# joncampbell123/composite-video-simulator

Measured on AMD Instinct MI355X. Metric: frames/sec (output frames = fields; 720x486 NTSC, preset '-vhs'; steady-state pipelined throughput, 4 steps in flight), higher is better.
Workload: dtype f64; 1 GPU; 720x486 30fps 10s colour-bars clip, preset '-vhs': 300 frames -> 600 fields per GPU per step, frame-round-robin over 1 GPU(s); steps_in_flight=4, mode=exact (bit-identical to the reference: fp64, no FMA contraction)

## Files before the change

### composite-video-simulator_amd/csrc/lane_rand.hpp

```cpp
#pragma once
#include <stdint.h>

#ifndef DEV
#define DEV __device__ __forceinline__
#endif

struct LaneRand {
    uint32_t p3, p2, p1;
    int slot;
    DEV void init(uint32_t *ring, const uint32_t *state, int stride, int lane)
    {
        for (int j = 0; j < 31; j++) ring[j * 64 + lane] = state[(size_t)j * stride];
        p3 = ring[28 * 64 + lane];
        p2 = ring[29 * 64 + lane];
        p1 = ring[30 * 64 + lane];
        slot = 0;
    }
    DEV uint32_t next(uint32_t *ring, int lane)
    {
#ifdef NTSC_AB_NORAND
        (void)ring; (void)lane;
        p3 = p3 * 1664525u + 1013904223u;
        return p3 >> 1;
#endif
        const uint32_t v = ring[slot * 64 + lane] + p3;
        ring[slot * 64 + lane] = v;
        p3 = p2; p2 = p1; p1 = v;
        slot = (slot == 30) ? 0 : slot + 1;
        return v >> 1;
    }
};

DEV void jump61(const uint32_t *__restrict__ c, const uint32_t *__restrict__ w, uint32_t (&o)[31])
{
    uint32_t cc[31], ww[61];
#pragma unroll
    for (int k = 0; k < 31; k++) cc[k] = c[k];
#pragma unroll
    for (int i = 0; i < 61; i++) ww[i] = w[i];
#pragma unroll
    for (int j = 0; j < 31; j++) {
        uint32_t acc = 0;
#pragma unroll
        for (int k = 0; k < 31; k++) acc += cc[k] * ww[j + k];
        o[j] = acc;
    }
}
```

### composite-video-simulator_amd/csrc/ntsc_device.hpp

```cpp
#pragma once
#include <cstdint>
#include "glibc_rand.hpp"

namespace ntscsim {

struct DevParams {
    int W, H;
    int Lslot;
    int nfields;
    int R;
    int Rpad;
    int ntsc;
    int phase_mode, phase_off;
    int in_lp;
    int out_lp;
    int amp, amp_back;
    Magic31 m_amp, m_amp_back;
    int noise_k;  Magic31 m_noise;
    int cnoise_k; Magic31 m_cnoise;
    int pnoise_k; Magic31 m_pnoise;
    int loss;
    int hs, hs_noise_on;
    double hs_point, hs_phase, hs_pn;
    int nocolor;
    int vhs, vblend, svideo, cdelay;
    int pre_on;
    double pre_gain, a_pre;
    double a_in_i, a_in_q, a_tv, a_vl, a_vc, a_sh;
    double sharpen;
    int src_al16, dst_al16;
    int warm_luma, warm_chroma;
    int variant;
    int ghost_taps, ghost_delay[4], ghost_gain[4];
};

struct FieldDev {
    const uint8_t *src;
    uint8_t *dst;
    int32_t src_ls, dst_ls;
    uint32_t field, flags;
    uint64_t fieldno;
    uint32_t rng[61];
    uint32_t _pad;
};
static_assert(sizeof(FieldDev) == 288, "FieldDev layout");

struct GeomDev {
    const uint32_t *lskip;
    const uint32_t *pskip;
    const uint32_t *jrow;
    const int32_t  *jwarm;
    const uint32_t *sstart;
    const double   *ptab;
};

}
```

### composite-video-simulator_amd/csrc/ntsc_kernels.hip

```cpp
#include <hip/hip_runtime.h>
#include <stdint.h>
#include "ntsc_device.hpp"

#pragma clang fp contract(off)

namespace ntscsim {

#define DEV __device__ __forceinline__

DEV int sdiv2(int n) { return (n + (int)((unsigned)n >> 31)) >> 1; }
DEV int sdiv4(int n) { return (n + ((n >> 31) & 3)) >> 2; }
DEV unsigned udiv31(unsigned n, const Magic31 &m) { return __umulhi(n, m.mul) >> m.shift; }
DEV unsigned umod31(unsigned n, const Magic31 &m) { return n - udiv31(n, m) * m.div; }
DEV int noise_next(int n, unsigned draw, const Magic31 &m, int k)
{
#ifdef NTSC_NOISE_UPDATE_OLD
    return sdiv2(n + (int)umod31(draw, m) - k);
#else
    int nk = -k;
    asm("" : "+s"(nk));
    unsigned t = ((unsigned)n + draw) + (unsigned)nk;
    asm("" : "+v"(t));
    return sdiv2((int)(t - udiv31(draw, m) * m.div));
#endif
}
DEV int sdivm(int n, const Magic31 &m)
{
    if (m.mul == 0) return n;
    const unsigned a = (unsigned)(n < 0 ? -n : n);
    const int q = (int)udiv31(a, m);
    return n < 0 ? -q : q;
}

DEV unsigned scan_phase(const DevParams &P, unsigned y, uint64_t fieldno)
{
// ... 123 lines not shown
            y += 2;
            shy++;
        }
    }

    if (P.pnoise_k || P.loss) {
        jump61(G.pskip + field * 31, fd.rng, st);
        g.init(ring, st, lane);
        if (P.pnoise_k) {
            int n = 0;
            for (int k = 0; k < L; k++) {
                n += (int)umod31(g.next(ring, lane), P.m_pnoise) - P.pnoise_k;
                n = sdiv2(n);
                pn_noise[(size_t)f * P.Lslot + k] = n;
            }
        }
        if (P.loss) {
            for (int k = 0; k < L; k++)
                dropout[(size_t)f * P.Lslot + k] = (g.next(ring, lane) % 100000U) < (unsigned)P.loss;
        }
    }
}

__global__ __launch_bounds__(64) void k_field_setup(DevParams P, GeomDev G,
                                                    const FieldDev *__restrict__ fields,
                                                    int *__restrict__ hs_shift,
                                                    int *__restrict__ pn_noise,
                                                    int *__restrict__ dropout)
{
    __shared__ uint32_t ring[31 * 64];
    field_setup_body(P, G, fields, hs_shift, pn_noise, dropout, ring, (int)blockIdx.x);
}

DEV void row_states_body(const DevParams &P, const GeomDev &G, const FieldDev *__restrict__ fields,
                         uint32_t *__restrict__ rs_luma, int *__restrict__ n0_luma,
                         uint32_t *__restrict__ rs_chroma, int *__restrict__ n0_u, int *__restrict__ n0_v,
                         uint32_t *ring, int block, int stream)
{
    const int lane = threadIdx.x;
    const int rho = block * 64 + lane;
    if (rho >= P.R) return;
    if (stream == 0 ? !P.noise_k : !P.cnoise_k) return;
    const int f = rho / P.Lslot, k = rho - f * P.Lslot;
    const FieldDev &fd = fields[f];
    const unsigned par = fd.field & 1u;
    if (k >= field_rows(P, par)) return;

    const size_t jidx = ((size_t)(stream * 2 + par) * P.Lslot + k);
    const int warm = G.jwarm[jidx];
    const int K = stream == 0 ? P.noise_k : P.cnoise_k;
    const Magic31 M = stream == 0 ? P.m_noise : P.m_cnoise;
    const long long cpr = P.variant ? 2ll * (P.W / 2) : 2ll * P.W;
    const long long start = stream == 0 ? (long long)k * P.W : cpr * k;
    const bool exact = (long long)warm == start;

    uint32_t st[31];
    SetupRand g;
    jump61(G.jrow + jidx * 31, fd.rng, st);
    g.init(ring, st, lane);

    int lo0 = exact ? 0 : -K, hi0 = exact ? 0 : K;
    int lo1 = stream == 0 ? 0 : lo0, hi1 = stream == 0 ? 0 : hi0;
    if (stream == 0) {
        for (int i = 0; i < warm; i++) {
            const int d = (int)umod31(g.next(ring, lane), M) - K;
            lo0 = sdiv2(lo0 + d); hi0 = sdiv2(hi0 + d);
        }
    } else {
        for (int i = 0; i < warm; i += 2) {
            int d = (int)umod31(g.next(ring, lane), M) - K;
            lo0 = sdiv2(lo0 + d); hi0 = sdiv2(hi0 + d);
            d = (int)umod31(g.next(ring, lane), M) - K;
            lo1 = sdiv2(lo1 + d); hi1 = sdiv2(hi1 + d);
        }
    }
    if (lo0 != hi0 || lo1 != hi1) {
        jump61(G.sstart + (size_t)(stream * 2 + par) * 31, fd.rng, st);
        g.init(ring, st, lane);
        lo0 = lo1 = 0;
        if (stream == 0) {
            for (long long i = 0; i < start; i++)
                lo0 = sdiv2(lo0 + (int)umod31(g.next(ring, lane), M) - K);
        } else {
            for (long long i = 0; i < start; i += 2) {
                lo0 = sdiv2(lo0 + (int)umod31(g.next(ring, lane), M) - K);
                lo1 = sdiv2(lo1 + (int)umod31(g.next(ring, lane), M) - K);
            }
        }
    }

    uint32_t *rs = stream == 0 ? rs_luma : rs_chroma;
    int q = g.slot;
    for (int j = 0; j < 31; j++) {
        rs[(size_t)j * P.Rpad + rho] = ring[q * 64 + lane];
        q = (q == 30) ? 0 : q + 1;
    }
    if (stream == 0) n0_luma[rho] = lo0;
    else { n0_u[rho] = lo0; n0_v[rho] = lo1; }
}

__global__ __launch_bounds__(64) void k_row_states(DevParams P, GeomDev G,
                                                   const FieldDev *__restrict__ fields,
                                                   uint32_t *__restrict__ rs_luma,
                                                   int *__restrict__ n0_luma,
                                                   uint32_t *__restrict__ rs_chroma,
                                                   int *__restrict__ n0_u, int *__restrict__ n0_v)
{
    __shared__ uint32_t ring[31 * 64];
    row_states_body(P, G, fields, rs_luma, n0_luma, rs_chroma, n0_u, n0_v, ring, (int)blockIdx.x, (int)blockIdx.y);
}

DEV void field_part_body(const DevParams &P, const GeomDev &G, const FieldDev *__restrict__ fields,
                         int *__restrict__ hs_shift, int *__restrict__ pn_noise, int *__restrict__ dropout,
                         uint32_t *ring, int f, int part)
{
    const int lane = threadIdx.x;
    const FieldDev &fd = fields[f];
    const unsigned field = fd.field & 1u;
    const int L = field_rows(P, field);
    const bool on = part == 0 ? P.hs != 0 : (part == 1 ? P.pnoise_k != 0 : P.loss != 0);
    if (!on) return;
    int *hs_row = hs_shift + (size_t)f * P.Lslot;
    if (part == 0)
        for (int k = lane; k < P.Lslot; k += 64) hs_row[k] = 0;
    if (part == 0) __builtin_amdgcn_s_waitcnt(0x0F70);
    if (part != 0 || P.hs_noise_on) {
        const uint32_t *c = (part == 0 ? G.lskip : G.pskip + (part == 2 ? 62 : 0)) + field * 31;
        if (lane < 31) {
            uint32_t acc = 0;
#pragma unroll
            for (int k = 0; k < 31; k++) acc += c[k] * fd.rng[lane + k];
// ... 789 lines not shown
```

### composite-video-simulator_amd/csrc/ntsc_key.hip

```cpp
#include <hip/hip_runtime.h>

#include <algorithm>
#include <cstdint>
#include <cstring>
#include <map>
#include <new>
#include <string>
#include <vector>

#include "key_host.hpp"
#include "ntscsim.h"
#include "ntsc_layer_frames.hpp"
#include "ntsc_px4.hpp"

namespace ntscsim {

#define KDEV __device__ __forceinline__

constexpr int KEY_FAST = NTSCSIM_KEY_FAST_LAYERS;
constexpr int KEY_THREADS = 256;
constexpr int KEY_DRAW_THREADS = 64;

struct KeyCfgLayer {
    uint32_t color;
    int32_t thr;
    uint32_t fade, xdivr, invert, noisekey;
};
struct KeyCfg { KeyCfgLayer l[KEY_FAST]; };

struct KeyLayerDev {
    const uint8_t *src;
    const uint32_t *bits;
    int32_t ls, _pad;
};

struct KeyRec {
    uint8_t *dst;
    const uint8_t *src[KEY_FAST];
    const uint32_t *bits[KEY_FAST];
    const KeyLayerDev *layers;
    int32_t src_ls[KEY_FAST];
    int32_t dst_ls;
    uint32_t vec;
    uint32_t _pad[2];
};

struct KeyJob {
    uint32_t st[31];
    uint32_t noisekey;
    uint32_t *bits;
};

struct KeyClip {
    uint8_t *const *ring;
    int32_t ring_ls, ri, delay, T;
};

#include "lane_rand.hpp"

__global__ __launch_bounds__(KEY_DRAW_THREADS) void k_key_draw(const KeyJob *__restrict__ jobs, const uint32_t *__restrict__ polys,
                                                               uint32_t lanes)
{
    __shared__ uint32_t ring[31 * 64];
    const int lane = threadIdx.x;
    const uint32_t j = blockIdx.x * KEY_DRAW_THREADS + lane;
    const uint32_t jj = j < lanes ? j : lanes - 1;
    const KeyJob &job = jobs[blockIdx.y];
    uint32_t w[61], c[31], st[31];
#pragma unroll
    for (int i = 0; i < 31; i++) w[i] = job.st[i];
#pragma unroll
    for (int i = 31; i < 61; i++) w[i] = w[i - 31] + w[i - 3];
#pragma unroll
    for (int k = 0; k < 31; k++) c[k] = polys[(size_t)k * lanes + jj];
    jump61(c, w, st);
#pragma unroll
    for (int i = 0; i < 31; i++) ring[i * 64 + lane] = st[i];
    LaneRand g;
    g.p3 = st[28]; g.p2 = st[29]; g.p1 = st[30];
    g.slot = 0;
    const uint32_t nk = job.noisekey;
    uint32_t *out = job.bits + (size_t)jj * KEY_RUN_WORDS;
#pragma unroll 1
    for (int wi = 0; wi < KEY_RUN_WORDS; wi++) {
        uint32_t word = 0;
#pragma unroll 4
        for (int b = 0; b < 32; b++) {
            const uint32_t r1 = g.next(ring, lane), r2 = g.next(ring, lane), r3 = g.next(ring, lane);
            const uint32_t x = (r1 * r2 * r3) % 20001u;
            word |= (x < nk ? 1u : 0u) << b;
// ... 596 lines not shown
```

### composite-video-simulator_amd/csrc/ntscsim_hip.hip

```cpp
#include <hip/hip_runtime.h>

#include <algorithm>
#include <cmath>
#include <cstdio>
#include <cstdlib>
#include <cstring>
#include <mutex>
#include <new>
#include <string>
#include <vector>

#include "ntscsim.h"
#include "ntsc_device.hpp"
#include "engine_host.hpp"

#include "ntsc_kernels.hip"
#include "ntsc_decode_fast.hip"
#include "ntsc_encode_fast.hip"
#include "ntsc_pipe.hip"
#include "ntsc422_kernels.hip"
#include "ntsc422_fused.hip"
#include "ntsc_scale.hip"
#include "ntsc_float.hpp"
#include "ntsc_stage.hpp"
// ... 20 lines not shown
        const hipError_t e = hipHostMalloc((void **)&bounce, CAP, hipHostMallocPortable);
        if (e != hipSuccess) { bounce = nullptr; return e; }
    }
    const unsigned char *s = static_cast<const unsigned char *>(src_host);
    unsigned char *d = static_cast<unsigned char *>(dst_dev);
    for (size_t off = 0; off < bytes; off += CAP) {
        const size_t n = bytes - off < CAP ? bytes - off : CAP;
        std::memcpy(bounce, s + off, n);
        const hipError_t e = hipMemcpy(d + off, bounce, n, hipMemcpyHostToDevice);
        if (e != hipSuccess) return e;
    }
    return hipSuccess;
}

template <typename T>
struct DevBuf {
    T *p = nullptr;
    size_t cap = 0;
    hipError_t ensure(size_t n)
    {
        if (n <= cap) return hipSuccess;
        if (p) { (void)hipFree(p); p = nullptr; cap = 0; }
        size_t want = n + n / 8 + 64;
        hipError_t e = hipMalloc((void **)&p, want * sizeof(T));
        if (e == hipSuccess) cap = want;
        return e;
    }
    void release() { if (p) (void)hipFree(p); p = nullptr; cap = 0; }
};

struct Geometry {
    int W = 0, H = 0, variant = 0;
    bool valid = false;
    DevBuf<uint32_t> lskip, pskip, jrow, sstart;
    DevBuf<int32_t> jwarm;
    uint64_t calls[2] = {0, 0};
};

}

struct SubmitEngine;
struct Host422Engine;
struct PinCache;

struct ntscsim_ctx {
    ntscsim_params prm;
    int device = 0;
    hipStream_t stream = nullptr;
    std::string err;
    uint64_t rng_pos = 0;

    bool have_state = false;
    uint64_t state_pos = 0;
    RandState state;
    struct Delta { uint64_t n; RandPoly p; };
    std::vector<Delta> deltas;

    std::vector<Geometry *> geoms;
    Geometry *geom_cur = nullptr;
    DevBuf<double> ptab;
    bool ptab_ready = false;

    DevBuf<FieldDev> fields;
    DevBuf<int> hs_shift, pn_noise, dropout, n0_luma, n0_u, n0_v, comp, comp_ghost, comp_vcr, tails;
    DevBuf<Field422Dev> fields422;
    DevBuf<uint8_t> recs422;
    DevBuf<uint32_t> scratch422;
    DevBuf<uint8_t> halo422;
// ... 143 lines not shown
    D.amp_back = p.subcarrier_amplitude_back;
    D.m_amp = magic31((uint32_t)D.amp);
    D.m_amp_back = magic31((uint32_t)D.amp_back);
    D.noise_k = p.video_noise;
    D.m_noise = magic31((uint32_t)(2 * p.video_noise + 1));
    D.cnoise_k = p.video_chroma_noise;
    D.m_cnoise = magic31((uint32_t)(2 * p.video_chroma_noise + 1));
    D.pnoise_k = p.video_chroma_phase_noise;
    D.m_pnoise = magic31((uint32_t)(2 * p.video_chroma_phase_noise + 1));
    D.loss = p.video_chroma_loss;
    D.hs = p.vhs_head_switching != 0;
    D.hs_noise_on = p.vhs_head_switching_phase_noise != 0;
    D.hs_point = p.vhs_head_switching_point;
    D.hs_phase = p.vhs_head_switching_phase;
    D.hs_pn = p.vhs_head_switching_phase_noise;
    D.nocolor = p.nocolor_subcarrier != 0;
    D.vhs = p.emulating_vhs != 0;
    D.vblend = p.vhs_chroma_vert_blend != 0;
    D.svideo = p.vhs_svideo_out != 0;
    double luma_cut = 2400000, chroma_cut = 320000;
    D.cdelay = 9;
    if (p.output_vhs_tape_speed == NTSCSIM_VHS_LP) { luma_cut = 1900000; chroma_cut = 300000; D.cdelay = 12; }
    if (p.output_vhs_tape_speed == NTSCSIM_VHS_EP) { luma_cut = 1400000; chroma_cut = 280000; D.cdelay = 14; }
    D.pre_on = (p.composite_preemphasis != 0 && p.composite_preemphasis_cut > 0);
    D.pre_gain = p.composite_preemphasis;
    D.a_pre = D.pre_on ? alpha_for(p.composite_preemphasis_cut) : 0;
    D.a_in_i = alpha_for(1300000);
    D.a_in_q = alpha_for(600000);
    D.a_tv = alpha_for(2600000);
    D.a_vl = alpha_for(luma_cut);
    D.a_vc = alpha_for(chroma_cut);
    D.a_sh = alpha_for(luma_cut * 4);
    D.sharpen = p.vhs_out_sharpen;
    D.warm_luma = 64;
    D.warm_chroma = 128;
    D.ghost_taps = p.ghost_taps;
    for (int k = 0; k < 4; k++) { D.ghost_delay[k] = p.ghost_delay[k]; D.ghost_gain[k] = p.ghost_gain[k]; }
}

static uint64_t chroma_stream_offset(const ntscsim_params &p, int W, int L)
{
    uint64_t o = 0;
    if (p.video_noise != 0) o += (uint64_t)W * L;
    if (p.vhs_head_switching && p.vhs_head_switching_phase_noise != 0) o += 4;
    return o;
}

static int build_geometry(ntscsim_ctx *c, int W, int H, const DevParams &D)
{
    for (Geometry *e : c->geoms)
        if (e->valid && e->W == W && e->H == H && e->variant == D.variant) { c->geom_cur = e; return NTSCSIM_OK; }
    if (c->geoms.size() >= 16) {
        HIPCHK(c, hipDeviceSynchronize());
        for (Geometry *e : c->geoms) {
            e->lskip.release(); e->pskip.release(); e->jrow.release(); e->sstart.release(); e->jwarm.release();
            delete e;
        }
        c->geoms.clear();
    }
    Geometry *gp = new (std::nothrow) Geometry();
    if (!gp) return NTSCSIM_E_NOMEM;
    c->geoms.push_back(gp);
    c->geom_cur = gp;
    Geometry &g = *gp;
    g.valid = false;
    const uint64_t cdraws = D.variant ? 2ull * (uint64_t)(W / 2) : 2ull * (uint64_t)W;
    const int Lslot = (H + 1) / 2;
    const int Lp[2] = {(H + 1) / 2, H / 2};
    std::vector<uint32_t> lskip(2 * 31), pskip(4 * 31), sstart(4 * 31), jrow((size_t)4 * Lslot * 31);
    std::vector<int32_t> jwarm((size_t)4 * Lslot);
    const RandPoly xW = rand_poly_pow((uint64_t)W), x2W = rand_poly_pow(cdraws);
    for (int par = 0; par < 2; par++) {
        const uint64_t off_hs = c->prm.video_noise != 0 ? (uint64_t)W * Lp[par] : 0;
        const uint64_t off_pn = chroma_stream_offset(c->prm, W, Lp[par]) +
                                (c->prm.video_chroma_noise != 0 ? cdraws * Lp[par] : 0);
        const RandPoly a = rand_poly_pow(off_hs);
        const RandPoly b = rand_poly_pow(off_pn);
        std::memcpy(&lskip[par * 31], a.c, sizeof(a.c));
        std::memcpy(&pskip[par * 31], b.c, sizeof(b.c));
        const RandPoly bd = rand_poly_pow(off_pn + (c->prm.video_chroma_phase_noise != 0 ? (uint64_t)Lp[par] : 0));
        std::memcpy(&pskip[(2 + par) * 31], bd.c, sizeof(bd.c));
        g.calls[par] = D.variant ? ntscsim_rng_calls_per_field_422(&c->prm, W, H, (unsigned)par)
                                 : ntscsim_rng_calls_per_field(&c->prm, W, H, (unsigned)par);
        for (int s = 0; s < 2; s++) {
            const uint64_t off = s == 0 ? 0 : chroma_stream_offset(c->prm, W, Lp[par]);
            const RandPoly so = rand_poly_pow(off);
            std::memcpy(&sstart[(size_t)(s * 2 + par) * 31], so.c, sizeof(so.c));
            const uint64_t warm_max = s == 0 ? (uint64_t)D.warm_luma : (uint64_t)D.warm_chroma;
            const uint64_t per_row = s == 0 ? (uint64_t)W : cdraws;
            const RandPoly &step = s == 0 ? xW : x2W;
            RandPoly cur = so;
            uint64_t cur_e = off;
            for (int k = 0; k < Lslot; k++) {
                const uint64_t start = per_row * (uint64_t)k;
                const uint64_t warm = start < warm_max ? start : warm_max;
                const uint64_t e = off + start - warm;
                if (e != cur_e) {
                    cur = (e - cur_e == per_row) ? rand_poly_mul(cur, step) : rand_poly_pow(e);
                    cur_e = e;
                }
                const size_t idx = (size_t)(s * 2 + par) * Lslot + k;
                std::memcpy(&jrow[idx * 31], cur.c, sizeof(cur.c));
                jwarm[idx] = (int32_t)warm;
            }
        }
    }
    HIPCHK(c, g.lskip.ensure(lskip.size()));
    HIPCHK(c, g.pskip.ensure(pskip.size()));
    HIPCHK(c, g.sstart.ensure(sstart.size()));
    HIPCHK(c, g.jrow.ensure(jrow.size()));
    HIPCHK(c, g.jwarm.ensure(jwarm.size()));
    HIPCHK(c, upload_table(g.lskip.p, lskip.data(), lskip.size() * 4));
    HIPCHK(c, upload_table(g.pskip.p, pskip.data(), pskip.size() * 4));
    HIPCHK(c, upload_table(g.sstart.p, sstart.data(), sstart.size() * 4));
    HIPCHK(c, upload_table(g.jrow.p, jrow.data(), jrow.size() * 4));
    HIPCHK(c, upload_table(g.jwarm.p, jwarm.data(), jwarm.size() * 4));
    g.W = W; g.H = H; g.variant = D.variant; g.valid = true;
    return NTSCSIM_OK;
}

static int build_ptab(ntscsim_ctx *c)
{
    if (c->ptab_ready) return NTSCSIM_OK;
    const int K = c->prm.video_chroma_phase_noise;
    std::vector<double> t((size_t)(2 * K + 1) * 2);
    for (int n = -K; n <= K; n++) {
        const double pi = ((double)n * M_PI) / 100;
        t[(size_t)(n + K) * 2] = std::cos(pi);
        t[(size_t)(n + K) * 2 + 1] = std::sin(pi);
    }
    HIPCHK(c, c->ptab.ensure(t.size()));
    HIPCHK(c, upload_table(c->ptab.p, t.data(), t.size() * sizeof(double)));
    c->ptab_ready = true;
    return NTSCSIM_OK;
}

extern "C" int ntscsim_create(const ntscsim_params *p, int device, ntscsim_ctx **out)
{
    if (!p || !out) return NTSCSIM_E_ARG;
    *out = nullptr;
    int rc = ntscsim_params_validate(p);
    if (rc != NTSCSIM_OK) return rc;
    int ndev = 0;
    if (hipGetDeviceCount(&ndev) != hipSuccess || ndev <= 0) return NTSCSIM_E_NODEV;
    if (device < 0 || device >= ndev) return NTSCSIM_E_NODEV;
    ntscsim_ctx *c = new (std::nothrow) ntscsim_ctx();
    if (!c) return NTSCSIM_E_NOMEM;
    c->prm = *p;
    c->device = device;
    if (const char *e = std::getenv("NTSCSIM_DEBUG_DECODE")) {
        const int v = std::atoi(e);
        c->no_fast_decode = (v & 1) != 0; c->split_vhs = (v & 2) != 0; c->no_stream422 = (v & 4) != 0;
        c->no_ghost_fuse = (v & 8) != 0; c->no_setup_merge = (v & 16) != 0;
    }
    if (hipSetDevice(device) != hipSuccess ||
        hipStreamCreateWithFlags(&c->stream, hipStreamNonBlocking) != hipSuccess) {
        delete c;
        return NTSCSIM_E_HIP;
    }
    for (int i = 0; i < 2; i++) (void)hipEventCreateWithFlags(&c->stage_ev[i], hipEventDisableTiming);
    for (int i = 0; i < 2; i++) (void)hipEventCreateWithFlags(&c->stage422_ev[i], hipEventDisableTiming);
    *out = c;
    return NTSCSIM_OK;
}

extern "C" void ntscsim_destroy(ntscsim_ctx *c)
{
    if (!c) return;
    (void)hipSetDevice(c->device);
    (void)hipDeviceSynchronize();
    submit_engine_destroy(c);
    host422_engine_destroy(c);
    declared_pins_destroy(c);
    if (c->blend) { ntscsim::blend_state_destroy(c->blend); c->blend = nullptr; }
    if (c->key) { ntscsim::key_state_destroy(c->key); c->key = nullptr; }
    if (c->avg) { ntscsim::avg_state_destroy(c->avg); c->avg = nullptr; }
    if (c->scan) { ntscsim::scan_state_destroy(c->scan); c->scan = nullptr; }
    for (Geometry *e : c->geoms) {
        e->lskip.release(); e->pskip.release(); e->jrow.release(); e->sstart.release(); e->jwarm.release();
        delete e;
    }
    c->geoms.clear();
    c->ptab.release(); c->fields.release(); c->hs_shift.release(); c->pn_noise.release();
    c->dropout.release(); c->n0_luma.release(); c->n0_u.release(); c->n0_v.release();
    c->comp.release(); c->comp_ghost.release(); c->comp_vcr.release(); c->tails.release(); c->fields422.release(); c->recs422.release(); c->out422.release(); c->yuv.release(); c->scale.release(); c->scratch422.release(); c->halo422.release(); c->rs_luma.release(); c->rs_chroma.release();
    c->fsrc.release(); c->fdst.release();
    for (auto &h : c->hslot) {
        h.dsrc.release(); h.ddst.release(); h.dyuv.release(); h.yrec.release(); h.draw.release(); h.srec.release();
        if (h.up) (void)hipEventDestroy(h.up);
        if (h.done) (void)hipEventDestroy(h.done);
        if (h.down) (void)hipEventDestroy(h.down);
    }
    if (c->ev_src) (void)hipEventDestroy(c->ev_src);
    if (c->ev_done) (void)hipEventDestroy(c->ev_done);
    if (c->spec.rec) (void)hipHostFree(c->spec.rec);
    c->alt.hs_shift.release(); c->alt.pn_noise.release(); c->alt.dropout.release(); c->alt.n0_luma.release();
    c->alt.n0_u.release(); c->alt.n0_v.release(); c->alt.rs_luma.release(); c->alt.rs_chroma.release();
    if (c->ev_spec) (void)hipEventDestroy(c->ev_spec);
    if (c->s_spec) (void)hipStreamDestroy(c->s_spec);
    if (std::getenv("NTSCSIM_SETUP_AHEAD_STATS") && c->spec.seen)
        std::fprintf(stderr, "setup ahead: %llu single-field launches, %llu early kernels, %llu used\n",
                     (unsigned long long)c->spec.seen, (unsigned long long)c->spec.launched, (unsigned long long)c->spec.hits);
    for (auto &e_ : c->ev_role) if (e_) (void)hipEventDestroy(e_);
    if (c->s_up) (void)hipStreamDestroy(c->s_up);
    if (c->s_dn) (void)hipStreamDestroy(c->s_dn);
    for (int i = 0; i < 2; i++) {
        if (c->stage[i]) (void)hipHostFree(c->stage[i]);
        if (i == 0 && c->pipe_fault) { (void)hipHostFree(c->pipe_fault); c->pipe_fault = nullptr; }
        if (c->stage_ev[i]) (void)hipEventDestroy(c->stage_ev[i]);
        if (c->stage422[i]) (void)hipHostFree(c->stage422[i]);
        if (c->stage422_ev[i]) (void)hipEventDestroy(c->stage422_ev[i]);
    }
// ... 57 lines not shown
extern "C" int ntscsim_set_mode(ntscsim_ctx *c, int mode)
{
    if (!c || (mode != NTSCSIM_MODE_EXACT && mode != NTSCSIM_MODE_FAST32 && mode != NTSCSIM_MODE_FLOAT)) return NTSCSIM_E_ARG;
    c->mode = mode;
    return NTSCSIM_OK;
}

extern "C" void ntscsim_debug_force_generic(ntscsim_ctx *c, int on)
{
    if (c) c->force_generic = on != 0;
}

extern "C" void ntscsim_debug_no_fast_decode(ntscsim_ctx *c, int on)
{
    if (c) { c->no_fast_decode = (on & 1) != 0; c->split_vhs = (on & 2) != 0; c->no_stream422 = (on & 4) != 0; c->no_ghost_fuse = (on & 8) != 0; c->no_setup_merge = (on & 16) != 0; }
}

extern "C" int ntscsim_debug_last_kernels(const ntscsim_ctx *c, char *out, size_t cap)
{
    if (!c || !out || cap == 0) return NTSCSIM_E_ARG;
    std::string kernels = c->kernels;
    if (c->scan) ntscsim::scan_kernels_tap(c->scan, c->device, kernels);
    const size_t n = std::min(cap - 1, kernels.size());
    std::memcpy(out, kernels.data(), n);
    out[n] = 0;
    return (int)kernels.size();
}

extern "C" void ntscsim_debug_set_warmup(ntscsim_ctx *c, int luma_draws, int chroma_draws)
{
    if (!c) return;
    c->warm_override[0] = luma_draws;
    c->warm_override[1] = chroma_draws & ~1;
    (void)hipSetDevice(c->device);
    (void)hipDeviceSynchronize();
    for (Geometry *e : c->geoms) e->valid = false;
}

#ifndef NTSC_SETUP_MERGE_MAX
#define NTSC_SETUP_MERGE_MAX 64
#endif
static void launch_setup_kernels(ntscsim_ctx *c, const DevParams &D, const GeomDev &G, const FieldDev *fields_dev, int n, hipStream_t st,
                                 bool note, bool launch)
{
    const bool fs = D.hs || D.pnoise_k || D.loss, rs = D.noise_k || D.cnoise_k;
    if (fs && rs && n <= NTSC_SETUP_MERGE_MAX && !c->no_setup_merge) {
        const int nfs = 3 * n, nrs = (D.R + 63) / 64;
        if (note) note_kernel(c, "k_field_row_setup");
        if (launch)
        hipLaunchKernelGGL(k_field_row_setup, dim3((unsigned)(nfs + 2 * nrs)), dim3(64), 0, st, D, G, fields_dev,
                           c->hs_shift.p, c->pn_noise.p, c->dropout.p, c->rs_luma.p, c->n0_luma.p, c->rs_chroma.p,
                           c->n0_u.p, c->n0_v.p, nfs, nrs);
        return;
    }
    if (fs) {
        if (note) note_kernel(c, "k_field_setup");
        if (launch)
        hipLaunchKernelGGL(k_field_setup, dim3((n + 63) / 64), dim3(64), 0, st, D, G, fields_dev,
                           c->hs_shift.p, c->pn_noise.p, c->dropout.p);
    }
    if (rs) {
        if (note) note_kernel(c, "k_row_states");
        if (launch)
        hipLaunchKernelGGL(k_row_states, dim3((D.R + 63) / 64, 2), dim3(64), 0, st, D, G,
                           fields_dev, c->rs_luma.p, c->n0_luma.p, c->rs_chroma.p, c->n0_u.p,
                           c->n0_v.p);
    }
}

// ... 162 lines not shown
    return span * Rpad * 4u < 0xFFF00000ull;
}

extern "C" int ntscsim_debug_fast_plane_ok(int n_fields, int W, int H, int head_switching)
{
    if (n_fields <= 0 || W <= 0 || H <= 0 || head_switching < 0 || head_switching > 2) return 0;
    const long long R = (long long)n_fields * ((H + 1) / 2);
    const size_t Rpad = (size_t)(((R + 63) / 64) * 64 + 64);
    return fast_plane_ok(Rpad, W, head_switching) ? 1 : 0;
}

static int launch_records(ntscsim_ctx *c, const DevParams &D, const FieldDev *fields_dev,
                          bool any_bob, hipStream_t st, const ntscsim_ctx::EvSet *evs)
{
    const int n = D.nfields, W = D.W, H = D.H;
    int grc = build_geometry(c, W, H, D);
    if (grc != NTSCSIM_OK) return grc;
    if (D.pnoise_k) { grc = build_ptab(c); if (grc != NTSCSIM_OK) return grc; }
    HIPCHK(c, c->comp.ensure((size_t)D.Rpad * W));
    if (D.hs) HIPCHK(c, c->hs_shift.ensure((size_t)D.R));
    if (D.pnoise_k) HIPCHK(c, c->pn_noise.ensure((size_t)D.R));
    if (D.loss) HIPCHK(c, c->dropout.ensure((size_t)D.R));
    if (D.noise_k) { HIPCHK(c, c->rs_luma.ensure((size_t)31 * D.Rpad)); HIPCHK(c, c->n0_luma.ensure((size_t)D.Rpad)); }
    if (D.cnoise_k) {
        HIPCHK(c, c->rs_chroma.ensure((size_t)31 * D.Rpad));
        HIPCHK(c, c->n0_u.ensure((size_t)D.Rpad));
        HIPCHK(c, c->n0_v.ensure((size_t)D.Rpad));
    }
    const dim3 dgrid((D.R + 62) / 63);
    if (D.vhs) HIPCHK(c, c->tails.ensure((size_t)32 * 64 * dgrid.x));

    GeomDev G;
    G.lskip = c->geom_cur->lskip.p; G.pskip = c->geom_cur->pskip.p; G.jrow = c->geom_cur->jrow.p;
    G.jwarm = c->geom_cur->jwarm.p; G.sstart = c->geom_cur->sstart.p; G.ptab = c->ptab.p;

    c->kernels.clear();
    launch_setup(c, D, G, fields_dev, n, st);
    if (c->src_pending) {
        c->src_pending = false;
        HIPCHK(c, hipStreamWaitEvent(st, c->ev_src, 0));
    }
    if (evs) HIPCHK(c, hipEventRecord(evs->e[1], st));
    static const bool role_probe = std::getenv("NTSCSIM_ROLE_PROBE") && std::getenv("NTSCSIM_ROLE_PROBE")[0] == '1';
    const bool enc_preset = !c->force_generic && D.in_lp && !D.pre_on && D.noise_k != 0 && D.amp == 50;
    const bool fast = c->mode != NTSCSIM_MODE_EXACT;
#define NTSC_LAUNCH_ENCODE(F, RT)                                                               \
    do { note_kernel(c, ("k_encode<" + std::to_string((unsigned)(F)) + "u," #RT ">").c_str());  \
    hipLaunchKernelGGL((k_encode<F, RT>), dim3((D.R + 63) / 64), dim3(64), 0, st, D,             \
                       fields_dev, c->rs_luma.p, c->n0_luma.p, c->comp.p); } while (0)
    const bool even_phase = (D.phase_mode == 180 || (D.phase_mode != 90 && D.phase_mode != 270)) && !(D.phase_off & 1);
    const bool hs_small = head_switch_is_small(D, W);
    const int hs_mode = !D.hs ? 0 : (hs_small ? 1 : 2);
    const bool small_plane = fast_plane_ok((size_t)D.Rpad, W, hs_mode);
    const bool enc_preset_pre = !c->force_generic && D.in_lp && D.pre_on && D.noise_k != 0 && D.amp == 50;
    bool ghost_fused = D.ghost_taps > 0 && !c->no_ghost_fuse;
    for (int k = 0; k < D.ghost_taps; k++) ghost_fused = ghost_fused && D.ghost_delay[k] < NTSC_GHOST_RING;
    ghost_fused = ghost_fused && enc_preset && !c->no_fast_decode && even_phase && small_plane && D.src_al16 &&
                  D.noise_k <= (1 << 20);
    const bool fp = c->mode == NTSCSIM_MODE_FLOAT && enc_preset && !c->no_fast_decode && even_phase && small_plane && D.src_al16 &&
                    D.ghost_taps == 0 && !D.nocolor && D.out_lp == 1 && D.amp == 50 && D.amp_back == 50 && D.dst_al16 && hs_small &&
                    !c->split_vhs &&
                    ((D.vhs && !D.svideo && D.cnoise_k && D.pnoise_k) || (!D.vhs && !D.cnoise_k && !D.pnoise_k));
    static const bool pipe_env = !(std::getenv("NTSCSIM_PIPE") && std::getenv("NTSCSIM_PIPE")[0] == '0');
    const bool pipe_xa = !even_phase && !D.svideo && fast_plane_ok((size_t)D.Rpad, W, D.hs ? 2 : 0);
    const bool pipe_catv = enc_preset_pre && D.amp_back != 50 && D.amp_back >= 2 && even_phase && !D.svideo &&
                           fast_plane_ok((size_t)D.Rpad, W, D.hs ? 2 : 0);
    static const bool pipe_always = std::getenv("NTSCSIM_PIPE_ALWAYS") && std::getenv("NTSCSIM_PIPE_ALWAYS")[0] == '1';
// ... 506 lines not shown

    P.any_render = any_render; P.any_flt = any_flt;
    P.rng_end = pos;
    return NTSCSIM_OK;
}

static int launch422(ntscsim_ctx *c, const Prep422 &P, const FieldDev *fields_dev, const Field422Dev *fields422_dev,
                     hipStream_t st, ntscsim_ctx::EvSet *evs)
{
    const ntscsim_params &p = c->prm;
    DevParams D = P.D;
    const int n = P.n, W = P.W, H = P.H;
    const bool any_render = P.any_render, any_flt = P.any_flt;
    const double a_hp_i = P.a_hp_i, a_hp_q = P.a_hp_q, a_sh_c = P.a_sh_c;
    int rc = build_geometry(c, W, H, D);
    if (rc != NTSCSIM_OK) return rc;
    if (D.pnoise_k) { rc = build_ptab(c); if (rc != NTSCSIM_OK) return rc; }
    const dim3 pgrid((D.R + 62) / 63);
    const size_t S = (size_t)pgrid.x * 64;
    const size_t W2 = (size_t)W / 2;
    const size_t Wq = ((size_t)W + 3) / 4 + 2, W2q = (W2 + 3) / 4 + 2;
    HIPCHK(c, c->scratch422.ensure(S * (2 * Wq + 2 * W2q) + 256));
    if (D.hs) HIPCHK(c, c->hs_shift.ensure((size_t)D.R));
    if (D.pnoise_k) HIPCHK(c, c->pn_noise.ensure((size_t)D.R));
    if (D.loss) HIPCHK(c, c->dropout.ensure((size_t)D.R));
    if (D.noise_k) { HIPCHK(c, c->rs_luma.ensure((size_t)31 * D.Rpad)); HIPCHK(c, c->n0_luma.ensure((size_t)D.Rpad)); }
    if (D.cnoise_k) {
        HIPCHK(c, c->rs_chroma.ensure((size_t)31 * D.Rpad));
        HIPCHK(c, c->n0_u.ensure((size_t)D.Rpad));
        HIPCHK(c, c->n0_v.ensure((size_t)D.Rpad));
    }
    GeomDev G;
    G.lskip = c->geom_cur->lskip.p; G.pskip = c->geom_cur->pskip.p; G.jrow = c->geom_cur->jrow.p;
    G.jwarm = c->geom_cur->jwarm.p; G.sstart = c->geom_cur->sstart.p; G.ptab = c->ptab.p;
    Scratch422 Sc;
    Sc.S = S;
    Sc.Y = c->scratch422.p;
    Sc.T = Sc.Y + S * Wq;
    Sc.U = Sc.T + S * Wq;
    Sc.V = Sc.U + S * W2q;
    Sc.halo_pitch = (uint32_t)((((size_t)P.max_ls + 2 + 63) / 64) * 64);
    Sc.halo = nullptr;
    if (pgrid.x > 1) {
        HIPCHK(c, c->halo422.ensure((size_t)pgrid.x * 3 * Sc.halo_pitch + 256));
        Sc.halo = c->halo422.p;
    }

    c->kernels.clear();
    if (any_render) note_kernel(c, "k422_render");
    if (any_flt) note_kernel(c, "k422_bkey");
    launch_setup(c, D, G, fields_dev, n, st);
    if (c->wait422_ev) {
        HIPCHK(c, hipStreamWaitEvent(st, c->wait422_ev, 0));
        c->wait422_ev = nullptr;
    }
    if (any_render)
        hipLaunchKernelGGL(k422_render, dim3((unsigned)((2 * W + 255) / 256), (unsigned)D.Lslot, (unsigned)n),
                           dim3(256), 0, st, D, fields422_dev);
    if (any_flt)
        hipLaunchKernelGGL(k422_bkey, dim3((unsigned)((W2 + 255) / 256), (unsigned)D.Lslot, (unsigned)n),
                           dim3(256), 0, st, D, fields422_dev, p.black_key_level_feedback);
    if (Sc.halo)
        hipLaunchKernelGGL(k422_halo, dim3(pgrid.x - 1), dim3(256), 0, st, D, fields422_dev, Sc);
    if (evs) { HIPCHK(c, hipEventRecord(evs->e[1], st)); HIPCHK(c, hipEventRecord(evs->e[2], st)); }
    const bool family = !c->no_fast_decode && !D.nocolor && D.in_lp &&
                        !p.nocolor_subcarrier_after_yc_sep && p.video_yc_recombine == 0;
    const bool fused = family && D.vhs && !D.svideo;
// ... 660 lines not shown
```

Measured before the change: 822,200 frames/s.

## Compute row noise state by backward RNG lookback instead of forward warm-up

Row-state setup now jumps the RNG directly to each row's start and recovers the noise accumulator from the last 24/31 draws already in the jumped state window. It only steps the lagged-additive generator backwards in extending chunks when the lower and upper bounds have not converged. This removes the 64/128-draw forward warm-up, the jwarm/sstart tables and the full-replay fallback. jump61 also switches to a v_mad_u64_u32 inline-asm accumulation. The cost is a more intricate convergence path that can still run longer backward replays for some rows.

```diff
diff --git a/composite-video-simulator_amd/csrc/lane_rand.hpp b/composite-video-simulator_amd/csrc/lane_rand.hpp
--- a/composite-video-simulator_amd/csrc/lane_rand.hpp
+++ b/composite-video-simulator_amd/csrc/lane_rand.hpp
@@ -40,9 +40,17 @@
     for (int i = 0; i < 61; i++) ww[i] = w[i];
 #pragma unroll
     for (int j = 0; j < 31; j++) {
+#ifndef NTSC_JUMP61_MUL_ADD
+        unsigned long long acc = 0, carry;
+#pragma unroll
+        for (int k = 0; k < 31; k++)
+            asm("v_mad_u64_u32 %0, %1, %2, %3, %0" : "+v"(acc), "=s"(carry) : "v"(cc[k]), "v"(ww[j + k]));
+        o[j] = (uint32_t)acc;
+#else
         uint32_t acc = 0;
 #pragma unroll
         for (int k = 0; k < 31; k++) acc += cc[k] * ww[j + k];
         o[j] = acc;
+#endif
     }
 }
diff --git a/composite-video-simulator_amd/csrc/ntsc_device.hpp b/composite-video-simulator_amd/csrc/ntsc_device.hpp
--- a/composite-video-simulator_amd/csrc/ntsc_device.hpp
+++ b/composite-video-simulator_amd/csrc/ntsc_device.hpp
@@ -49,8 +49,6 @@
     const uint32_t *lskip;
     const uint32_t *pskip;
     const uint32_t *jrow;
-    const int32_t  *jwarm;
-    const uint32_t *sstart;
     const double   *ptab;
 };
 
diff --git a/composite-video-simulator_amd/csrc/ntsc_kernels.hip b/composite-video-simulator_amd/csrc/ntsc_kernels.hip
--- a/composite-video-simulator_amd/csrc/ntsc_kernels.hip
+++ b/composite-video-simulator_amd/csrc/ntsc_kernels.hip
@@ -1,6 +1,7 @@
 #include <hip/hip_runtime.h>
 #include <stdint.h>
 #include "ntsc_device.hpp"
+#include "ntsc_rowstate_lookback.hpp"
 
 #pragma clang fp contract(off)
 
@@ -190,6 +191,30 @@
     field_setup_body(P, G, fields, hs_shift, pn_noise, dropout, ring, (int)blockIdx.x);
 }
 
+template <bool CHROMA>
+DEV void row_lookback(const DevParams &P, const uint32_t (&st)[31], uint32_t *ring, int lane, long long start,
+                      rowstate::Acc &a)
+{
+    constexpr int M0 = CHROMA ? rowstate::LOOK_CHROMA : rowstate::LOOK_LUMA;
+    const int K = CHROMA ? P.cnoise_k : P.noise_k;
+    const Magic31 M = CHROMA ? P.m_cnoise : P.m_noise;
+    const int m0 = CHROMA ? P.warm_chroma : P.warm_luma;
+    const bool window = m0 == M0 && !__builtin_amdgcn_ballot_w64(start != 0 && start < M0);
+    bool open = true;
+    if (window) {
+        rowstate::from_window<M0, CHROMA>(st, M, K, start <= M0, a);
+        if (start == 0) a.init(true, CHROMA, K);
+        open = !a.settled();
+    }
+    if (!__builtin_amdgcn_ballot_w64(open)) return;
+    rowstate::Ring r;
+    r.col = ring + lane; r.stride = 64;
+    r.load(st);
+    const long long m = rowstate::clip(start, m0);
+    if (!window) rowstate::replay(r, m, start, CHROMA, M, K, a);
+    (void)rowstate::extend(r, m, start, CHROMA, M, K, a);
+}
+
 DEV void row_states_body(const DevParams &P, const GeomDev &G, const FieldDev *__restrict__ fields,
                          uint32_t *__restrict__ rs_luma, int *__restrict__ n0_luma,
                          uint32_t *__restrict__ rs_chroma, int *__restrict__ n0_u, int *__restrict__ n0_v,
@@ -205,56 +230,20 @@
     if (k >= field_rows(P, par)) return;
 
     const size_t jidx = ((size_t)(stream * 2 + par) * P.Lslot + k);
-    const int warm = G.jwarm[jidx];
-    const int K = stream == 0 ? P.noise_k : P.cnoise_k;
-    const Magic31 M = stream == 0 ? P.m_noise : P.m_cnoise;
     const long long cpr = P.variant ? 2ll * (P.W / 2) : 2ll * P.W;
     const long long start = stream == 0 ? (long long)k * P.W : cpr * k;
-    const bool exact = (long long)warm == start;
 
     uint32_t st[31];
-    SetupRand g;
     jump61(G.jrow + jidx * 31, fd.rng, st);
-    g.init(ring, st, lane);
-
-    int lo0 = exact ? 0 : -K, hi0 = exact ? 0 : K;
-    int lo1 = stream == 0 ? 0 : lo0, hi1 = stream == 0 ? 0 : hi0;
-    if (stream == 0) {
-        for (int i = 0; i < warm; i++) {
-            const int d = (int)umod31(g.next(ring, lane), M) - K;
-            lo0 = sdiv2(lo0 + d); hi0 = sdiv2(hi0 + d);
-        }
-    } else {
-        for (int i = 0; i < warm; i += 2) {
-            int d = (int)umod31(g.next(ring, lane), M) - K;
-            lo0 = sdiv2(lo0 + d); hi0 = sdiv2(hi0 + d);
-            d = (int)umod31(g.next(ring, lane), M) - K;
-            lo1 = sdiv2(lo1 + d); hi1 = sdiv2(hi1 + d);
-        }
-    }
-    if (lo0 != hi0 || lo1 != hi1) {
-        jump61(G.sstart + (size_t)(stream * 2 + par) * 31, fd.rng, st);
-        g.init(ring, st, lane);
-        lo0 = lo1 = 0;
-        if (stream == 0) {
-            for (long long i = 0; i < start; i++)
-                lo0 = sdiv2(lo0 + (int)umod31(g.next(ring, lane), M) - K);
-        } else {
-            for (long long i = 0; i < start; i += 2) {
-                lo0 = sdiv2(lo0 + (int)umod31(g.next(ring, lane), M) - K);
-                lo1 = sdiv2(lo1 + (int)umod31(g.next(ring, lane), M) - K);
-            }
-        }
-    }
+    rowstate::Acc a;
+    if (stream == 0) row_lookback<false>(P, st, ring, lane, start, a);
+    else row_lookback<true>(P, st, ring, lane, start, a);
 
     uint32_t *rs = stream == 0 ? rs_luma : rs_chroma;
-    int q = g.slot;
-    for (int j = 0; j < 31; j++) {
-        rs[(size_t)j * P.Rpad + rho] = ring[q * 64 + lane];
-        q = (q == 30) ? 0 : q + 1;
-    }
-    if (stream == 0) n0_luma[rho] = lo0;
-    else { n0_u[rho] = lo0; n0_v[rho] = lo1; }
+#pragma unroll
+    for (int j = 0; j < 31; j++) rs[(size_t)j * P.Rpad + rho] = st[j];
+    if (stream == 0) n0_luma[rho] = a.lo0;
+    else { n0_u[rho] = a.lo0; n0_v[rho] = a.lo1; }
 }
 
 __global__ __launch_bounds__(64) void k_row_states(DevParams P, GeomDev G,
diff --git a/composite-video-simulator_amd/csrc/ntsc_key.hip b/composite-video-simulator_amd/csrc/ntsc_key.hip
--- a/composite-video-simulator_amd/csrc/ntsc_key.hip
+++ b/composite-video-simulator_amd/csrc/ntsc_key.hip
@@ -56,6 +56,7 @@
     int32_t ring_ls, ri, delay, T;
 };
 
+#define NTSC_JUMP61_MUL_ADD
 #include "lane_rand.hpp"
 
 __global__ __launch_bounds__(KEY_DRAW_THREADS) void k_key_draw(const KeyJob *__restrict__ jobs, const uint32_t *__restrict__ polys,
diff --git a/composite-video-simulator_amd/csrc/ntsc_rowstate_lookback.hpp b/composite-video-simulator_amd/csrc/ntsc_rowstate_lookback.hpp
--- /dev/null
+++ b/composite-video-simulator_amd/csrc/ntsc_rowstate_lookback.hpp
@@ -0,0 +1,109 @@
+#pragma once
+#include <stdint.h>
+#include "glibc_rand.hpp"
+
+#ifdef __HIPCC__
+#define NTSC_LB_FN __host__ __device__ __forceinline__
+#else
+#define NTSC_LB_FN inline
+#endif
+
+namespace ntscsim {
+namespace rowstate {
+
+constexpr int LOOK_LUMA = 24;
+constexpr int LOOK_CHROMA = 31;
+constexpr int EXTEND = 32;
+
+NTSC_LB_FN int half(int n) { return (n + (int)((unsigned)n >> 31)) >> 1; }
+NTSC_LB_FN unsigned mulhi(unsigned a, unsigned b)
+{
+#ifdef __HIP_DEVICE_COMPILE__
+    return __umulhi(a, b);
+#else
+    return (unsigned)(((unsigned long long)a * b) >> 32);
+#endif
+}
+NTSC_LB_FN int delta(uint32_t word, const Magic31 &M, int K)
+{
+    const unsigned draw = word >> 1;
+    return (int)(draw - (mulhi(draw, M.mul) >> M.shift) * M.div) - K;
+}
+
+struct Acc {
+    int lo0, hi0, lo1, hi1;
+    NTSC_LB_FN void init(bool exact, bool chroma, int K)
+    {
+        lo0 = exact ? 0 : -K; hi0 = exact ? 0 : K;
+        lo1 = chroma ? lo0 : 0; hi1 = chroma ? hi0 : 0;
+    }
+    NTSC_LB_FN void push0(int d) { lo0 = half(lo0 + d); hi0 = half(hi0 + d); }
+    NTSC_LB_FN void push1(int d) { lo1 = half(lo1 + d); hi1 = half(hi1 + d); }
+    NTSC_LB_FN bool settled() const { return lo0 == hi0 && lo1 == hi1; }
+};
+
+template <int M0, bool CHROMA>
+NTSC_LB_FN void from_window(const uint32_t (&st)[31], const Magic31 &M, int K, bool exact, Acc &a)
+{
+    static_assert(M0 >= 1 && M0 <= 31, "the window holds 31 draws");
+    a.init(exact, CHROMA, K);
+#ifdef __HIPCC__
+#pragma unroll
+#endif
+    for (int i = M0; i >= 1; i--) {
+        const int d = delta(st[31 - i], M, K);
+        if (CHROMA && (i & 1)) a.push1(d); else a.push0(d);
+    }
+}
+
+struct Ring {
+    uint32_t *col;
+    int stride;
+    int slot;
+    NTSC_LB_FN void load(const uint32_t (&st)[31])
+    {
+        for (int j = 0; j < 31; j++) col[j * stride] = st[j];
+        slot = 0;
+    }
+    NTSC_LB_FN void back()
+    {
+        const int n = slot == 0 ? 30 : slot - 1;
+        const int j = n >= 3 ? n - 3 : n + 28;
+        col[n * stride] -= col[j * stride];
+        slot = n;
+    }
+    NTSC_LB_FN uint32_t fwd()
+    {
+        const int j = slot >= 3 ? slot - 3 : slot + 28;
+        const uint32_t v = col[slot * stride] + col[j * stride];
+        col[slot * stride] = v;
+        slot = slot == 30 ? 0 : slot + 1;
+        return v;
+    }
+};
+
+NTSC_LB_FN void replay(Ring &r, long long m, long long start, bool chroma, const Magic31 &M, int K, Acc &a)
+{
+    for (long long i = 0; i < m; i++) r.back();
+    a.init(m == start, chroma, K);
+    for (long long i = 0; i < m; i++) {
+        const int d = delta(r.fwd(), M, K);
+        if (chroma && ((m + i) & 1)) a.push1(d); else a.push0(d);
+    }
+}
+
+NTSC_LB_FN long long clip(long long start, int m0) { return start < (long long)m0 ? start : (long long)m0; }
+
+NTSC_LB_FN int extend(Ring &r, long long m, long long start, bool chroma, const Magic31 &M, int K, Acc &a)
+{
+    int rounds = 0;
+    while (!a.settled() && m < start) {
+        m = start - m < (long long)EXTEND ? start : m + EXTEND;
+        replay(r, m, start, chroma, M, K, a);
+        rounds++;
+    }
+    return rounds;
+}
+
+}
+}
diff --git a/composite-video-simulator_amd/csrc/ntscsim_hip.hip b/composite-video-simulator_amd/csrc/ntscsim_hip.hip
--- a/composite-video-simulator_amd/csrc/ntscsim_hip.hip
+++ b/composite-video-simulator_amd/csrc/ntscsim_hip.hip
@@ -76,8 +76,7 @@
 struct Geometry {
     int W = 0, H = 0, variant = 0;
     bool valid = false;
-    DevBuf<uint32_t> lskip, pskip, jrow, sstart;
-    DevBuf<int32_t> jwarm;
+    DevBuf<uint32_t> lskip, pskip, jrow;
     uint64_t calls[2] = {0, 0};
 };
 
@@ -287,8 +286,8 @@
     D.a_vc = alpha_for(chroma_cut);
     D.a_sh = alpha_for(luma_cut * 4);
     D.sharpen = p.vhs_out_sharpen;
-    D.warm_luma = 64;
-    D.warm_chroma = 128;
+    D.warm_luma = rowstate::LOOK_LUMA;
+    D.warm_chroma = rowstate::LOOK_CHROMA;
     D.ghost_taps = p.ghost_taps;
     for (int k = 0; k < 4; k++) { D.ghost_delay[k] = p.ghost_delay[k]; D.ghost_gain[k] = p.ghost_gain[k]; }
 }
@@ -308,7 +307,7 @@
     if (c->geoms.size() >= 16) {
         HIPCHK(c, hipDeviceSynchronize());
         for (Geometry *e : c->geoms) {
-            e->lskip.release(); e->pskip.release(); e->jrow.release(); e->sstart.release(); e->jwarm.release();
+            e->lskip.release(); e->pskip.release(); e->jrow.release();
             delete e;
         }
         c->geoms.clear();
@@ -322,8 +321,7 @@
     const uint64_t cdraws = D.variant ? 2ull * (uint64_t)(W / 2) : 2ull * (uint64_t)W;
     const int Lslot = (H + 1) / 2;
     const int Lp[2] = {(H + 1) / 2, H / 2};
-    std::vector<uint32_t> lskip(2 * 31), pskip(4 * 31), sstart(4 * 31), jrow((size_t)4 * Lslot * 31);
-    std::vector<int32_t> jwarm((size_t)4 * Lslot);
+    std::vector<uint32_t> lskip(2 * 31), pskip(4 * 31), jrow((size_t)4 * Lslot * 31);
     const RandPoly xW = rand_poly_pow((uint64_t)W), x2W = rand_poly_pow(cdraws);
     for (int par = 0; par < 2; par++) {
         const uint64_t off_hs = c->prm.video_noise != 0 ? (uint64_t)W * Lp[par] : 0;
@@ -340,36 +338,27 @@
         for (int s = 0; s < 2; s++) {
             const uint64_t off = s == 0 ? 0 : chroma_stream_offset(c->prm, W, Lp[par]);
             const RandPoly so = rand_poly_pow(off);
-            std::memcpy(&sstart[(size_t)(s * 2 + par) * 31], so.c, sizeof(so.c));
-            const uint64_t warm_max = s == 0 ? (uint64_t)D.warm_luma : (uint64_t)D.warm_chroma;
             const uint64_t per_row = s == 0 ? (uint64_t)W : cdraws;
             const RandPoly &step = s == 0 ? xW : x2W;
             RandPoly cur = so;
             uint64_t cur_e = off;
             for (int k = 0; k < Lslot; k++) {
-                const uint64_t start = per_row * (uint64_t)k;
-                const uint64_t warm = start < warm_max ? start : warm_max;
-                const uint64_t e = off + start - warm;
+                const uint64_t e = off + per_row * (uint64_t)k;
                 if (e != cur_e) {
                     cur = (e - cur_e == per_row) ? rand_poly_mul(cur, step) : rand_poly_pow(e);
                     cur_e = e;
                 }
                 const size_t idx = (size_t)(s * 2 + par) * Lslot + k;
                 std::memcpy(&jrow[idx * 31], cur.c, sizeof(cur.c));
-                jwarm[idx] = (int32_t)warm;
             }
         }
     }
     HIPCHK(c, g.lskip.ensure(lskip.size()));
     HIPCHK(c, g.pskip.ensure(pskip.size()));
-    HIPCHK(c, g.sstart.ensure(sstart.size()));
     HIPCHK(c, g.jrow.ensure(jrow.size()));
-    HIPCHK(c, g.jwarm.ensure(jwarm.size()));
     HIPCHK(c, upload_table(g.lskip.p, lskip.data(), lskip.size() * 4));
     HIPCHK(c, upload_table(g.pskip.p, pskip.data(), pskip.size() * 4));
-    HIPCHK(c, upload_table(g.sstart.p, sstart.data(), sstart.size() * 4));
     HIPCHK(c, upload_table(g.jrow.p, jrow.data(), jrow.size() * 4));
-    HIPCHK(c, upload_table(g.jwarm.p, jwarm.data(), jwarm.size() * 4));
     g.W = W; g.H = H; g.variant = D.variant; g.valid = true;
     return NTSCSIM_OK;
 }
@@ -432,7 +421,7 @@
     if (c->avg) { ntscsim::avg_state_destroy(c->avg); c->avg = nullptr; }
     if (c->scan) { ntscsim::scan_state_destroy(c->scan); c->scan = nullptr; }
     for (Geometry *e : c->geoms) {
-        e->lskip.release(); e->pskip.release(); e->jrow.release(); e->sstart.release(); e->jwarm.release();
+        e->lskip.release(); e->pskip.release(); e->jrow.release();
         delete e;
     }
     c->geoms.clear();
@@ -556,9 +545,6 @@
     if (!c) return;
     c->warm_override[0] = luma_draws;
     c->warm_override[1] = chroma_draws & ~1;
-    (void)hipSetDevice(c->device);
-    (void)hipDeviceSynchronize();
-    for (Geometry *e : c->geoms) e->valid = false;
 }
 
 #ifndef NTSC_SETUP_MERGE_MAX
@@ -787,7 +773,7 @@
 
     GeomDev G;
     G.lskip = c->geom_cur->lskip.p; G.pskip = c->geom_cur->pskip.p; G.jrow = c->geom_cur->jrow.p;
-    G.jwarm = c->geom_cur->jwarm.p; G.sstart = c->geom_cur->sstart.p; G.ptab = c->ptab.p;
+    G.ptab = c->ptab.p;
 
     c->kernels.clear();
     launch_setup(c, D, G, fields_dev, n, st);
@@ -1360,7 +1346,7 @@
     }
     GeomDev G;
     G.lskip = c->geom_cur->lskip.p; G.pskip = c->geom_cur->pskip.p; G.jrow = c->geom_cur->jrow.p;
-    G.jwarm = c->geom_cur->jwarm.p; G.sstart = c->geom_cur->sstart.p; G.ptab = c->ptab.p;
+    G.ptab = c->ptab.p;
     Scratch422 Sc;
     Sc.S = S;
     Sc.Y = c->scratch422.p;
```

Measured after the change: 832,800 frames/s (median of 6 runs). 1.3% higher.
